# BiaPyX/BiaPy

Hardware: AMD Instinct MI355X
Metric: voxels/sec 3D ResUNet 128^3 patch (train: fwd+bwd+AdamW; sub-records: infer, sliding) (higher is better)
Workload: dtype f16 forward/activations + bf16 gradients (MFMA f16 / bf16, fp32 accumulate)

## Files before the change

biapy_amd/_lib.py:

```python
from __future__ import annotations

import ctypes as C
import os
from typing import Optional

import torch

_HERE = os.path.dirname(os.path.abspath(__file__))
LIB_PATH = os.environ.get("BPX_LIB_PATH") or os.path.join(_HERE, "libbiapy_amd.so")

F32, BF16, F16, U8, MIX16 = 0, 1, 2, 3, 4
U16 = 5
I32 = 6
ACT = {"none": 0, "linear": 0, "elu": 1, "relu": 2, "silu": 3, "leaky_relu": 4, "gelu": 5, "tanh": 6, "sigmoid": 7, "softplus": 8}
PK_K3, PK_K3_T, PK_K1, PK_DENSE, PK_DENSE_T, PK_CT, PK_CT_T, PK_CT4, PK_CT4_T = range(9)


class AxisGrid(C.Structure):
    _fields_ = [("n", C.c_int32), ("step", C.c_int32), ("last", C.c_int32), ("patch", C.c_int32), ("limit", C.c_int32)]


class Tensor(C.Structure):
    _fields_ = [("ptr", C.c_void_p), ("ld", C.c_int32), ("C", C.c_int32), ("cs", C.c_int64)]

# ... 104 lines not shown
    "bpx_debug_set_wgrad_k1": ([_i], _i),
    "bpx_debug_set_pw_stream": ([_i], _i),
    "bpx_debug_set_convt_k1": ([_i], _i),
    "bpx_debug_set_c1_persist": ([_i], _i),
    "bpx_convT3d_k2s2_wgrad_workspace": ([_i, _i, _i, _i, _i, _i, _i], _i64),
    "bpx_conv1x1_fwd": ([_i, _i, _i64, Tensor, _vp, _vp, Tensor, Tensor, _vp, Tensor, Tensor, _vp], _i),
    "bpx_conv1x1_fwd_split_wgrad_workspace": ([_i, _i, _i64, _i], _i64),
    "bpx_conv1x1_fwd_split_wgrad_query": ([_i, _i, _i64, Tensor, Tensor, Tensor, _vp, Tensor, Tensor], _i64),
    "bpx_conv1x1_fwd_split_wgrad": ([_i, _i, _i64, Tensor, _vp, Tensor, Tensor, _vp, Tensor, Tensor, _vp, _vp, _i64, _vp], _i),
    "bpx_conv1x1_fwd_split": ([_i, _i, _i64, Tensor, _vp, _vp, Tensor, Tensor, _vp, Tensor, Tensor, Tensor, _vp], _i),
    "bpx_convT3d_k2s2_fwd": ([_i, _i, _i, _i, _i, _i, Tensor, _vp, _vp, Tensor, _vp, _vp], _i),
    "bpx_convT3d_stats_tiles": ([_i, _i, _i, _i], _i),
    "bpx_convT3d_k2s2_dgrad": ([_i, _i, _i, _i, _i, _i, Tensor, _vp, Tensor, _vp], _i),
    "bpx_convT3d_k2s2_wgrad": ([_i, _i, _i, _i, _i, _i, Tensor, Tensor, _vp, _vp, _vp, _i64, _vp], _i),
    "bpx_convT3d_k2s2_bwd": ([_i, _i, _i, _i, _i, _i, Tensor, Tensor, _vp, Tensor, _vp, _vp, _vp, _i64, _vp], _i),
    "bpx_debug_set_convt_bwd": ([_i], _i),
    "bpx_debug_convt_bwd_launches": ([], _i),
    "bpx_norm_finalize": ([_vp, _i, _i, _i, _i64, _vp, _vp, _f, _i, _vp, _i, _i, _vp], _i),
    "bpx_norm_channel_sums": ([_vp, _i, _i, _i, _vp, _i, _i, _vp], _i),
    "bpx_groupnorm_finalize": ([_vp, _i, _i, _i64, _vp, _vp, _f, _i, _vp, _vp], _i),
    "bpx_groupnorm_bwd_finalize": ([_vp, _i, _i, _i64, _vp, _vp, _vp, _vp, _i, _vp, _vp], _i),
    "bpx_tensor_stats": ([_i, _i, _i64, Tensor, _vp, _vp], _i),
    "bpx_tensor_stats_tiles": ([_i64], _i),
    "bpx_norm_bwd_finalize": ([_vp, _i, _i, _i, _i64, _vp, _vp, _vp, _vp, _i, _vp, _vp], _i),
    "bpx_norm_bwd_finalize_deferred": ([_vp, _i, _i, _i, _i64, _vp, _vp, _vp, _vp, _i, _vp, _vp], _i),
    "bpx_batchnorm_finalize": ([_vp, _i, _i, _i, _i64, _vp, _vp, _f, _f, _vp, _vp, _vp, _vp, _i, _i, _vp], _i),
    "bpx_batchnorm_bwd_finalize": ([_vp, _i, _i, _i, _i64, _vp, _vp, _vp, _vp, _i, _vp, _vp], _i),
    "bpx_batchnorm_eval_records": ([_i, _vp, _i, _vp], _i),
    "bpx_gather3d_tables": ([_vp, _i, _i, _i, _i, _i, _vp, _i, _i, _i, _i, _vp, _vp], _i),
    "bpx_scatter3d_tables": ([_vp, _i, _vp, _i, _i, _i, _i, _vp, _i, _i, _i, _i, _vp], _i),
    "bpx_scatter3d_regions": ([_vp, _i, _i, _i, _i, _i, _vp, _vp, _i, _i, _i, _vp], _i),
    "bpx_wgrad_defer_begin": ([], _i),
    "bpx_wgrad_defer_flush": ([_vp], _i),
    "bpx_norm_bwd_apply": ([_i, _i, _i64, Tensor, Tensor, _vp, Tensor, Tensor, _vp], _i),
    "bpx_channel_affine": ([_i, _i, _i64, Tensor, Tensor, _vp, _vp, Tensor, _vp], _i),
    "bpx_dot_stats": ([_i, _i, _i64, Tensor, Tensor, _vp, _vp], _i),
    "bpx_gate_mlp_fwd": ([_vp, _i, _i, _i, _i64, _vp, _vp, _vp, _vp, _i, _i, _vp, _vp, _vp], _i),
    "bpx_gate_mlp_bwd": ([_vp, _i, _i, _i, _i64, _vp, _vp, _vp, _vp, _i, _i, _vp, _vp, _vp, _vp, _vp, _vp], _i),
    "bpx_norm_act_tiles": ([_i, _i64, _i], _i),
    "bpx_norm_act_dropout_tiles": ([_i, _i64, _i], _i),
    "bpx_norm_act_dropout_fwd": ([_i, _i, _i64, Tensor, _vp, _i, C.c_float, C.c_uint64, _vp, _i, _vp, _i, Tensor, _vp], _i),
    "bpx_norm_act_dropout_bwd": ([_i, _i, _i64, Tensor, Tensor, _vp, _i, C.c_float, C.c_uint64, _vp, _i, _vp, _i, Tensor, _vp, _vp], _i),
    "bpx_norm_act_fwd": ([_i, _i, _i64, Tensor, _vp, _i, Tensor, _vp], _i),
    "bpx_norm_act_bwd": ([_i, _i, _i64, Tensor, Tensor, _vp, _i, Tensor, Tensor, _vp, _vp], _i),
    "bpx_maxpool3d_fwd": ([_i, _i, _i, _i, _i, _i, Tensor, Tensor, _vp, _vp], _i),
    "bpx_maxpool3d_stats_tiles": ([_i, _i, _i, _i, _i, _i], _i),
    "bpx_maxpool3d_bwd_r1_workspace": ([_i, _i, _i, _i, _i, _i, _i], _i64),
    "bpx_maxpool3d_bwd_r1": ([_i, _i, _i, _i, _i, _i, Tensor, Tensor, Tensor, Tensor, _vp, _vp, _vp, _i64, _vp], _i),
    "bpx_maxpool3d_bwd": ([_i, _i, _i, _i, _i, _i, Tensor, Tensor, Tensor, Tensor, _vp], _i),
    "bpx_head_fwd": ([_i, _i64, _i, Tensor, _vp, _vp, _i, _i, _vp, _i64, _i64, _vp], _i),
    "bpx_head_bwd": ([_i, _i64, _i, Tensor, _vp, _i, _vp, _i64, _i64, Tensor, _vp, _vp, _vp, _i64, _vp], _i),
    "bpx_head_bwd_workspace": ([_i, _i], _i64),
    "bpx_conv3d_c1_wgrad_workspace": ([_i], _i64),
    "bpx_conv1x1_c1_wgrad_workspace": ([_i], _i64),
    "bpx_conv3d_c1_fwd": ([_i, _i, _i, _i, _i, _vp, _vp, _vp, Tensor, _vp, _vp], _i),
    "bpx_conv3d_c1_stats_tiles": ([_i, _i, _i], _i),
    "bpx_conv3d_c1_wgrad": ([_i, _i, _i, _i, _i, _vp, Tensor, _vp, _vp, _vp, _i64, _vp], _i),
    "bpx_conv3d_c1_wgrad_nb_supported": ([_i, _i], _i),
    "bpx_conv3d_c1_wgrad_nb": ([_i, _i, _i, _i, _i, _vp, Tensor, Tensor, _vp, _vp, _vp, _vp, _i64, _vp], _i),
    "bpx_conv1x1_c1_wgrad": ([_i, _i64, _vp, Tensor, _vp, _vp, _i64, _vp], _i),
    "bpx_cast": ([_i, _vp, _i, _vp, _i64, _vp], _i),
    "bpx_image_pack16": ([_i, _i, _i64, _i, _vp, _i64, _i64, _i64, _vp, _vp], _i),
    "bpx_upsample_c1_fwd": ([_i, _i, _i, _i, _i, _i, _i, _i, _vp, _vp, _vp, _vp, _vp], _i),
    "bpx_upsample_c1_blocks": ([_i64], _i),
    "bpx_upsample_c1_bwd": ([_i, _i, _i, _i, _i, _i, _i, _i, _vp, _vp, _vp, _vp], _i),
}

EXPORTS = tuple(_SIGS.keys())


class BpxError(RuntimeError):
    pass


def _load() -> C.CDLL:
    if not os.path.exists(LIB_PATH):
        raise ImportError(
            f"{LIB_PATH} is missing: the HIP extension is the product and there is no fallback. "
            "Build it with `python -c 'import __graft_entry__ as g; g.build()'` or `make -C biapy_amd/csrc`."
        )
    lib = C.CDLL(LIB_PATH)
    for name, (args, res) in _SIGS.items():
        fn = getattr(lib, name)
        fn.argtypes = args
        fn.restype = res
    for env, hook in (("BPX_WGRAD_CAP", "bpx_debug_set_wgrad_cap"), ("BPX_WGRAD_K1", "bpx_debug_set_wgrad_k1"),
                      ("BPX_PW_STREAM", "bpx_debug_set_pw_stream"), ("BPX_C1_PERSIST", "bpx_debug_set_c1_persist"),
                      ("BPX_BWD_RS", "bpx_debug_set_bwd_rs"), ("BPX_FUSED_BITS", "bpx_debug_set_bwd_fused"),
                      ("BPX_CT_BWD", "bpx_debug_set_convt_bwd"), ("BPX_LABEL_TILED", "bpx_debug_set_label_tiled"),
                      ("BPX_OVERLAP_PER_VOXEL", "bpx_debug_set_overlap_per_voxel"),
                      ("BPX_REGIONPROPS_LOCAL", "bpx_debug_set_regionprops_local")):
        if os.environ.get(env) is not None:
            getattr(lib, hook)(int(os.environ[env]))
    return lib


class PackJob(C.Structure):
    _fields_ = [("w_d", C.c_void_p), ("packed_d", C.c_void_p), ("mode", C.c_int32), ("Cin", C.c_int32), ("Cout", C.c_int32),
                ("reserved", C.c_int32)]


class BnEvalJob(C.Structure):
    _fields_ = [("gamma_d", C.c_void_p), ("beta_d", C.c_void_p), ("running_mean_d", C.c_void_p), ("running_var_d", C.c_void_p), ("out_d", C.c_void_p),
                ("C", C.c_int32), ("eps", C.c_float)]


class AugCfg(C.Structure):
    _fields_ = [("seed", C.c_uint64), ("thr", C.c_uint64), ("enable", C.c_uint32), ("box_lo", C.c_int32), ("box_hi", C.c_int32),
                ("c_lo", C.c_float), ("c_hi", C.c_float), ("b_lo", C.c_float), ("b_hi", C.c_float), ("s_lo", C.c_float), ("s_hi", C.c_float),
                ("f_lo", C.c_float), ("f_hi", C.c_float)]


class WarpCfg(C.Structure):
    _fields_ = [("seed", C.c_uint64), ("thr", C.c_uint64), ("enable", C.c_uint32), ("reserved", C.c_uint32), ("rot_lo", C.c_float),
                ("rot_hi", C.c_float), ("zoom_lo", C.c_float), ("zoom_hi", C.c_float), ("shear_lo", C.c_float), ("shear_hi", C.c_float),
                ("shift_lo", C.c_float), ("shift_hi", C.c_float)]


class PatchVol(C.Structure):
    _fields_ = [("img", C.c_void_p), ("tgt", C.c_void_p), ("cls", C.c_void_p), ("Z", C.c_int32), ("Y", C.c_int32), ("X", C.c_int32),
                ("reserved", C.c_int32), ("row0", C.c_int64)]

# ... 135 lines not shown
```

biapy_amd/csrc/bpx_common.h:

```cpp
#pragma once
#include <hip/hip_runtime.h>
#include <stdint.h>
#include <stdio.h>
#include <string.h>

#include "../../include/biapy_amd.h"

void bpx_set_error(const char* fmt, ...);
#define BPX_FAIL(...)            \
  do {                           \
    bpx_set_error(__VA_ARGS__);  \
    return 1;                    \
  } while (0)
#define BPX_CHECK(cond, ...) \
  do {                       \
    if (!(cond)) BPX_FAIL(__VA_ARGS__); \
  } while (0)
#define BPX_LAUNCH_CHECK(name)                                                         \
  do {                                                                                 \
    hipError_t e__ = hipGetLastError();                                                \
    if (e__ != hipSuccess) BPX_FAIL("%s: launch failed: %s", name, hipGetErrorString(e__)); \
  } while (0)

typedef __attribute__((ext_vector_type(8))) short bf16x8_t;
// ... 168 lines not shown
  return v;
}

template <int ACTK> __device__ __forceinline__ void act_pair(float& a, float& b, int act) {
  if (ACTK == 1) {
    f32x2_t u{a, b};
    f32x2_t w = u * f32x2_t{1.44269504088896341f, 1.44269504088896341f};
    f32x2_t e = f32x2_t{__builtin_amdgcn_exp2f(w[0]), __builtin_amdgcn_exp2f(w[1])} + f32x2_t{-1.f, -1.f};
    a = __builtin_amdgcn_fmed3f(u[0], e[0], 0.f);
    b = __builtin_amdgcn_fmed3f(u[1], e[1], 0.f);
  } else {
    a = bpx_act_rt<false, false>(a, act);
    b = bpx_act_rt<false, false>(b, act);
  }
}

template <typename T> __device__ __forceinline__ f32x4_t mfma_step(const u32x4_t& a, const u32x4_t& b, f32x4_t c);
template <> __device__ __forceinline__ f32x4_t mfma_step<uint16_t>(const u32x4_t& a, const u32x4_t& b, f32x4_t c) {
  return __builtin_amdgcn_mfma_f32_16x16x32_bf16(__builtin_bit_cast(bf16x8_t, a), __builtin_bit_cast(bf16x8_t, b), c, 0, 0, 0);
}
template <> __device__ __forceinline__ f32x4_t mfma_step<f16_t>(const u32x4_t& a, const u32x4_t& b, f32x4_t c) {
  return __builtin_amdgcn_mfma_f32_16x16x32_f16(__builtin_bit_cast(f16x8_t, a), __builtin_bit_cast(f16x8_t, b), c, 0, 0, 0);
}
template <> __device__ __forceinline__ f32x4_t mfma_step<float>(const u32x4_t& a, const u32x4_t& b, f32x4_t c) {
#pragma unroll
  for (int j = 0; j < 4; ++j)
    c = __builtin_amdgcn_mfma_f32_16x16x4f32(__uint_as_float(a[j]), __uint_as_float(b[j]), c, 0, 0, 0);
  return c;
}

__host__ __device__ __forceinline__ int64_t cdiv64(int64_t a, int64_t b) { return (a + b - 1) / b; }
__host__ __device__ __forceinline__ int cdiv(int a, int b) { return (a + b - 1) / b; }

static inline size_t dtype_size(int dt) {
  switch (dt) {
    case BPX_F32: return 4;
    case BPX_BF16: case BPX_F16: return 2;
    case BPX_U8: return 1;
  }
  return 0;
}

namespace bpxred {
bool defer_active();
int reduce_rows(const char* fn, const float* rows, int groups, int64_t stride, int n, float* dst, hipStream_t s);
int reduce_partials(const char* fn, const float* part, float* dw, int groups, int taps, int Cin, int Cout, int64_t si, int64_t sj, int64_t st,
                    const float* dbpart, float* db, int ndb, bool may_defer, hipStream_t s);
int reduce_partials2(const char* fn, const float* part, float* dw, int groups, int taps, int Cin, int Cout, int64_t si, int64_t sj, int64_t st,
                     const float* dbpart, float* db, float* db2, int ndb, bool may_defer, hipStream_t s);
}
```

biapy_amd/csrc/bwd_fused.hip:

```cpp
#include "conv3d_shared.h"
#include "wgrad_shared.h"

using namespace bpxconv;

#ifndef BPX_BWD_OCC1
#define BPX_BWD_OCC1 3
#endif
#ifndef BPX_BWD_LDSW
#define BPX_BWD_LDSW 1
#endif
#ifndef BPX_BWD_RS_WPRIO
#define BPX_BWD_RS_WPRIO 1
#endif

namespace {

#ifdef BPX_TICKET_PROBE
__device__ unsigned g_probe_ticket = 0u, g_probe_last = 0u;
#endif
struct BwdParams {
  int N, D, H, W;
  const void* dy; int dy_ld;
  const void* wT;
  const void* t; int t_ld; int t_cs; int Ct;
// ... 859 lines not shown
      q_live = have;
      BPX_STAMP();
#pragma unroll
      for (int q = 0; q < NP; ++q) piece(q);
      __builtin_amdgcn_sched_barrier(0);
      BPX_STAMP();
      bpxwg::sd_mfma_phase<WW, CT, HY, HX, VB, VB, TV, NKC>(sA, sG, a_base, g_lane, accw[0], want_b);
      BPX_STAMP();
      if (lane == 0) __hip_atomic_fetch_add(wsync, 1u, __ATOMIC_RELAXED, __HIP_MEMORY_SCOPE_WORKGROUP);
    }
    float* pp = p.part + (size_t)blockIdx.x * 27 * Ct * 16;
#pragma unroll
    for (int a = 0; a < 7; ++a) {
      const int tap = 7 * WW + a;
      if (tap >= 27) continue;
#pragma unroll
      for (int c = 0; c < CT; ++c)
#pragma unroll
        for (int r = 0; r < 4; ++r) pp[((size_t)tap * Ct + c * 16 + 4 * g + r) * 16 + j] = accw[0][a][c][r];
    }
    if (want_b && WW == 3 && g == 0) p.dbpart[(size_t)blockIdx.x * 16 + j] = accw[0][6][0][0];
    __builtin_amdgcn_s_waitcnt(0x0F70);
    };
    switch (ww) {
      case 0: w_role(std::integral_constant<int, 0>{}); break;
      case 1: w_role(std::integral_constant<int, 1>{}); break;
      case 2: w_role(std::integral_constant<int, 2>{}); break;
      default: w_role(std::integral_constant<int, 3>{}); break;
    }
  }
#undef BPX_STAMP
}

int cu_count_() {
  static int n = 0;
  if (n == 0) {
    int dev = 0, v = 0;
    if (hipGetDevice(&dev) == hipSuccess && hipDeviceGetAttribute(&v, hipDeviceAttributeMultiprocessorCount, dev) == hipSuccess && v > 0) n = v;
    else n = 256;
  }
  return n;
}

int g_bwd_fused = 1;

#ifndef BPX_BWD_RS_DEFAULT
#define BPX_BWD_RS_DEFAULT 3
#endif
int g_bwd_rs = BPX_BWD_RS_DEFAULT;

struct BwdPlan { int cg, ct, gy, grid, tilesZ, tilesY, tilesX; bool per_wg_rows; bool rs; };
bool bwd_instance(int Ct, int Cdy, BwdPlan& q) {
  q.gy = 1;
  if (Cdy == 16 && Ct == 16) { q.cg = 1; q.ct = 1; }
  else if (Cdy == 16 && Ct == 48) { q.cg = 1; q.ct = 3; }
  else if (Cdy == 32 && (Ct == 16 || Ct == 32)) { q.cg = 2; q.ct = 1; q.gy = Ct / 16; }
  else return false;
  q.rs = q.cg == 1 && ((q.ct == 3 && (g_bwd_rs & 1)) || (q.ct == 1 && (g_bwd_rs & 2)));
  q.per_wg_rows = q.rs || !(q.cg == 1 && q.ct == 3);
  return true;
}
BwdPlan bwd_plan(int N, int D, int H, int W, int Ct, int Cdy) {
  BwdPlan q{};
  bwd_instance(Ct, Cdy, q);
  q.tilesZ = cdiv(D, 4); q.tilesY = cdiv(H, 4); q.tilesX = cdiv(W, 16);
  const int total = N * q.tilesZ * q.tilesY * q.tilesX;
  const int occ = q.rs ? (q.ct == 1 ? 2 : 1) : (q.cg == 1 && q.ct == 1) ? BPX_BWD_OCC1 : 2;
  int gx = std::max(8, (cu_count_() * occ / std::max(1, q.gy)) & ~7);
  gx = std::min(gx, 8 * cdiv(total, 8));
  q.grid = gx;
  return q;
}

int g_bwd_level1 = 1;

// ... 89 lines not shown
```

biapy_amd/csrc/wgrad.hip:

```cpp
#include <algorithm>
#include <type_traits>
#include <vector>

#include "conv3d_shared.h"
#include "wgrad_shared.h"

namespace {
using bpxwg::sd_mfma_phase;

struct WgradParams {
  int N, D, H, W;
  const void* x; int x_ld; int Cin; const bpx_norm_rec* in_norm; int act;
  int x_cs;
  int x_f16;
  const void* dy; int dy_ld; int Cout; int dy_vs; int dy_oz, dy_oy, dy_ox;
  int dy_vz;
  float* part;
  float* dw; int64_t si, sj, st; int64_t off;
  float* db;
  float* dbpart;
  float* db2;
  int tilesY, tilesX, tilesPerSample, totalTiles, groups;
  int tilesZ, stripY, order;
  void* dx; int dx_ld; const void* wT;
// ... 904 lines not shown
}

int g_ct_resident = 1;
struct CtCfg { int ns, groups, totalTiles, tilesY, tilesX, tilesPerSample; };
inline int ct_mc(int N, int D, int H, int W, int sz, int Cin, int Cout) {
  static const int env = getenv("BPX_CT_MC") ? atoi(getenv("BPX_CT_MC")) : 2;
  return (env >= 2 && sz == 2 && (Cin / 16) % 2 == 0 && Cout % 32 == 0 && (int64_t)N * D * H * W >= 262144) ? 2 : 1;
}
inline CtCfg pick_ct(int N, int D, int H, int W, int sz, int Cin, int Cout) {
  CtCfg c;
  c.ns = (Cout % 32 == 0) ? 2 : 1;
  c.tilesY = cdiv(H, 4); c.tilesX = cdiv(W, 16);
  c.tilesPerSample = cdiv(D, 2) * c.tilesY * c.tilesX;
  c.totalTiles = N * c.tilesPerSample;
  const int nchunks = Cin / (16 * ct_mc(N, D, H, W, sz, Cin, Cout)), nb = Cout / (16 * c.ns);
  const int64_t cap = std::max<int64_t>(1, (int64_t)6400000 / ((int64_t)4 * sz * Cin * Cout));
  const int occ = c.ns == 1 ? 4 : 2;
  const int64_t want = g_ct_resident ? (cdiv64((int64_t)256 * occ, nchunks * nb) + 7) & ~7ll : std::max(1, cdiv(2048, nchunks * nb));
  c.groups = (int)std::max<int64_t>(1, std::min<int64_t>(std::min<int64_t>(c.totalTiles, cap), want));
  return c;
}

struct ReduceJob { const float* part; float* dw; int groups, taps, Cin, Cout; int64_t si, sj, st, off; const float* dbpart; float* db; int ndb; float* db2 = nullptr; int64_t db_stride = 0; };

__host__ __device__ inline int reduce_glanes(int groups) {
  int gl = 1;
  while (gl < 32 && gl * 4 < groups) gl <<= 1;
  return gl;
}
inline int reduce_blocks(const ReduceJob& j) {
  return (int)cdiv64((int64_t)j.taps * j.Cin * j.Cout + (j.db ? (j.ndb ? j.ndb : j.Cout) : 0), 4 * (1024 / reduce_glanes(j.groups)));
}

__device__ __forceinline__ void wgrad_reduce_block(const ReduceJob& j, int block) {
  __shared__ f32x4_t red[1024];
  const float* __restrict__ part = j.part;
  const int groups = j.groups;
  const int GL = reduce_glanes(groups), EL = 1024 / GL;
  const int ndb = j.ndb ? j.ndb : j.Cout;
  const int64_t total = (int64_t)j.taps * j.Cin * j.Cout, all = total + (j.db ? ndb : 0);
  const int e = threadIdx.x % EL, gl = threadIdx.x / EL;
  const int64_t idx = ((int64_t)block * EL + e) * 4;
  const float* __restrict__ src = idx < total ? part + idx : j.dbpart + (idx - total);
  const int64_t stride = idx < total ? total : (j.db_stride ? j.db_stride : ndb);
  const int nval = idx >= all ? 0 : (int)(all - idx < 4 ? all - idx : 4);
  const bool vec = nval == 4 && (stride & 3) == 0 && (((uintptr_t)src) & 15) == 0;
  f32x4_t s0 = f32x4_t{0.f, 0.f, 0.f, 0.f}, s1 = s0, s2 = s0, s3 = s0;
  if (vec) {
    int gq = gl;
    for (; gq + 3 * GL < groups; gq += 4 * GL) {
      s0 += *reinterpret_cast<const f32x4_t*>(src + (size_t)gq * stride);
      s1 += *reinterpret_cast<const f32x4_t*>(src + (size_t)(gq + GL) * stride);
      s2 += *reinterpret_cast<const f32x4_t*>(src + (size_t)(gq + 2 * GL) * stride);
      s3 += *reinterpret_cast<const f32x4_t*>(src + (size_t)(gq + 3 * GL) * stride);
    }
    for (; gq < groups; gq += GL) s0 += *reinterpret_cast<const f32x4_t*>(src + (size_t)gq * stride);
  } else if (nval > 0) {
    int gq = gl;
    for (; gq + 3 * GL < groups; gq += 4 * GL) {
      float a[4][4];
#pragma unroll
      for (int u = 0; u < 4; ++u)
#pragma unroll
        for (int k = 0; k < 4; ++k) a[u][k] = k < nval ? src[(size_t)(gq + u * GL) * stride + k] : 0.f;
#pragma unroll
      for (int u = 0; u < 4; ++u)
#pragma unroll
        for (int k = 0; k < 4; ++k) if (k < nval) s0[k] += a[u][k];
    }
    for (; gq < groups; gq += GL)
      for (int k = 0; k < nval; ++k) s0[k] += src[(size_t)gq * stride + k];
  }
  red[gl * EL + e] = (s0 + s1) + (s2 + s3);
  __syncthreads();
  if (gl == 0 && nval > 0) {
    f32x4_t s = red[e];
    for (int q = 1; q < GL; ++q) s += red[q * EL + e];
    for (int k = 0; k < nval; ++k) {
      const int64_t i = idx + k;
      if (i < total) {
        int co = (int)(i % j.Cout), ci = (int)((i / j.Cout) % j.Cin), tap = (int)(i / ((int64_t)j.Cout * j.Cin));
        j.dw[ci * j.si + co * j.sj + tap * j.st + j.off] = s[k];
      } else {
        j.db[i - total] += s[k];
        if (j.db2) j.db2[i - total] += s[k];
      }
    }
  }
}

__global__ void __launch_bounds__(1024) wgrad_reduce_kernel(const ReduceJob j) { wgrad_reduce_block(j, (int)blockIdx.x); }

constexpr int RB_MAX = 32;
struct ReduceBatch { ReduceJob job[RB_MAX]; int first_block[RB_MAX + 1]; int count; };
__global__ void __launch_bounds__(1024) wgrad_reduce_batch_kernel(const ReduceBatch b) {
  int lo = 0, hi = b.count;
  while (hi - lo > 1) {
    const int mid = (lo + hi) >> 1;
    if ((int)blockIdx.x >= b.first_block[mid]) lo = mid; else hi = mid;
  }
  wgrad_reduce_block(b.job[lo], (int)blockIdx.x - b.first_block[lo]);
}

struct DeferState { bool active = false; std::vector<ReduceJob> jobs; };
thread_local DeferState t_defer;

int finish_wgrad(const char* fn, const ReduceJob& j, hipStream_t s) {
  if (t_defer.active) { t_defer.jobs.push_back(j); return 0; }
  wgrad_reduce_kernel<<<reduce_blocks(j), 1024, 0, s>>>(j);
  BPX_LAUNCH_CHECK(fn);
  return 0;
}

struct K1Params {
  const void* x; int x_ld; int x_cs; const void* dy; int dy_ld;
  int Cin, Cout; int64_t voxels; int nblocks; int groups; float* part;
};
__host__ __device__ constexpr int k1_ring(int stage_bytes) { return 4 * stage_bytes <= 131072 ? 4 : 3 * stage_bytes <= 131072 ? 3 : 2; }
__host__ __device__ constexpr int vmcnt_imm(int n) { return (n & 15) | ((n >> 4) << 14) | 0x0F70; }

template <int MC, int NS, int TV, bool XF16>
__global__ void __launch_bounds__(256) wgrad_k1_dma_kernel(const K1Params p) {
  constexpr int VB = 32, SUBS = TV / 32;
  constexpr int A_BYTES = MC * TV * VB, STAGE = (MC + NS) * TV * VB, RING = k1_ring(STAGE);
  constexpr int NI = (MC + NS) * SUBS;
  static_assert(NI % 4 == 0, "every wave issues the same number of DMA instructions per stage");
  constexpr int IPW = NI / 4;
  static_assert((RING - 2) * IPW < 64, "vmcnt range");
  __shared__ __attribute__((aligned(16))) unsigned char smem[RING * STAGE];
  typedef __attribute__((address_space(3))) void* lds_ptr_t;
  typedef __attribute__((address_space(3))) s16x4_t* lds_tr_ptr;
  const int tid = threadIdx.x, lane = tid & 63, wave = tid >> 6;
  const int i = lane & 15, g = lane >> 4;
  const int grp = blockIdx.x;
  const __amdgpu_buffer_rsrc_t rs_x = __builtin_amdgcn_make_buffer_rsrc(const_cast<void*>(p.x), 0, (int)0x80000000u, 0x00020000);
  const __amdgpu_buffer_rsrc_t rs_g = __builtin_amdgcn_make_buffer_rsrc(const_cast<void*>(p.dy), 0, (int)0x80000000u, 0x00020000);
  const uint32_t xvb = (uint32_t)p.x_ld * 2u, gvb = (uint32_t)p.dy_ld * 2u, xcb = (uint32_t)p.x_cs * 2u;
  const uint32_t lane_v = (uint32_t)(lane >> 1), lane_h = (uint32_t)(lane & 1) * 16u;
  const int64_t voxels = p.voxels;
  const int groups = p.groups, nblocks = p.nblocks;
// ... 412 lines not shown
    BPX_LAUNCH_CHECK(fn);
    return finish_wgrad(fn, ReduceJob{p.part, p.dw, groups, 1, p.Cin, p.Cout, p.si, p.sj, p.st, p.off, nullptr, nullptr, 0, nullptr}, s);
  }
  int rc;
  const int64_t vox = (int64_t)p.N * p.D * p.H * p.W;
  const bool sd_ok = dtype == BPX_BF16 && taps == 27 && p.dy_vs == 1 && c.tx == 16 && c.tz == 4 && g_use_tr != 0 &&
                     vox * std::max(p.x_ld, p.dy_ld) < (1ll << 31) && (((uintptr_t)p.in_norm) & 7) == 0 &&
                     !(p.in_norm != nullptr && p.act > BPX_ACT_SILU);
  if (sd_ok && g_wgrad_sd != 0) rc = launch_wgrad_sd(p, c, s);
  else if (dtype == BPX_BF16) rc = (taps == 27) ? launch_wgrad<uint16_t, 27>(p, c, g_use_tr != 0, s) : launch_wgrad<uint16_t, 1>(p, c, g_use_tr != 0, s);
  else rc = (taps == 27) ? launch_wgrad<float, 27>(p, c, false, s) : launch_wgrad<float, 1>(p, c, false, s);
  BPX_CHECK(rc == 0, "%s: no kernel for tile config", fn);
  BPX_LAUNCH_CHECK(fn);
  const float* dbpart = p.db ? p.part + (size_t)c.groups * taps * p.Cin * p.Cout : nullptr;
  return finish_wgrad(fn, ReduceJob{p.part, p.dw, c.groups, taps, p.Cin, p.Cout, p.si, p.sj, p.st, p.off, dbpart, p.db, 0, p.db ? p.db2 : nullptr}, s);
}

}

namespace bpxred {
int reduce_partials(const char* fn, const float* part, float* dw, int groups, int taps, int Cin, int Cout, int64_t si, int64_t sj, int64_t st,
                    const float* dbpart, float* db, int ndb, bool may_defer, hipStream_t s) {
  return reduce_partials2(fn, part, dw, groups, taps, Cin, Cout, si, sj, st, dbpart, db, nullptr, ndb, may_defer, s);
}
bool defer_active() { return t_defer.active; }
int reduce_rows(const char* fn, const float* rows, int groups, int64_t stride, int n, float* dst, hipStream_t s) {
  ReduceJob j{nullptr, nullptr, groups, 0, 0, n, 0, 0, 0, 0, rows, dst, n, nullptr, stride};
  return finish_wgrad(fn, j, s);
}
int reduce_partials2(const char* fn, const float* part, float* dw, int groups, int taps, int Cin, int Cout, int64_t si, int64_t sj, int64_t st,
                     const float* dbpart, float* db, float* db2, int ndb, bool may_defer, hipStream_t s) {
  const ReduceJob j{part, dw, groups, taps, Cin, Cout, si, sj, st, 0, db ? dbpart : nullptr, db, ndb, db ? db2 : nullptr};
  if (may_defer) return finish_wgrad(fn, j, s);
  wgrad_reduce_kernel<<<reduce_blocks(j), 1024, 0, s>>>(j);
  BPX_LAUNCH_CHECK(fn);
  return 0;
}
}

extern "C" int64_t bpx_conv3d_wgrad_workspace(int N, int D, int H, int W, int Cin, int Cout, int k) {
  int taps = k * k * k;
  WCfg c = pick_wcfg(N, D, H, W, Cin, Cout, taps, false);
  int64_t groups = c.groups;
  if (taps == 27) groups = std::max<int64_t>(groups, sdm_plan(N, D, H, W, Cin, Cout).groups);
  if (taps == 1) groups = std::max<int64_t>(groups, 256);
  return groups * ((int64_t)taps * Cin + 1) * Cout * 4;
}
extern "C" int64_t bpx_convT3d_k2s2_wgrad_workspace(int N, int D, int H, int W, int sz, int Cin, int Cout) {
  WCfg c = pick_wcfg(N, D, H, W, Cin, Cout, 1, false);
  CtCfg t = pick_ct(N, D, H, W, sz, Cin, Cout);
  return std::max(std::max((int64_t)c.groups * ((int64_t)Cin + 1) * Cout * 4, (int64_t)t.groups * ((int64_t)4 * sz * Cin + 1) * Cout * 4),
                  (int64_t)256 * ((int64_t)4 * sz * Cin + 1) * Cout * 4);
}

extern "C" int bpx_debug_set_wgrad_tr(int use_tr) {
  g_use_tr = use_tr & 1;
  g_wgrad_sd = (use_tr & 4) ? 1 : (use_tr & 2) ? 0 : -1;
  g_sd_mc = ((use_tr >> 3) & 7) == 4 ? 0 : ((use_tr >> 3) & 3) ? ((use_tr >> 3) & 3) : -1;
  g_ct_resident = ((use_tr >> 6) & 1) ? 0 : 1;
  if ((use_tr >> 7) & 1) { g_k1_wgs = 1024 * (use_tr >> 8) / 100; g_sd_fill = 100; }
  else g_sd_fill = (use_tr >> 8) ? (use_tr >> 8) : 100;
  return 0;
}

extern "C" int bpx_debug_set_tile_order(int bits) { g_sd_order = bits & 1; return 0; }

// ... 120 lines not shown
    p.dw = dw_d; p.si = (int64_t)dy.C * nsub; p.sj = nsub; p.st = 0; p.off = sub;
    p.db = db_d;
    if (run_wgrad(fn, dtype, p, 1, ws_d, ws_bytes, (hipStream_t)stream)) return 1;
  }
  return 0;
}

}

extern "C" int bpx_convT3d_k2s2_wgrad(int dtype, int N, int D, int H, int W, int sz, bpx_tensor x, bpx_tensor dy, float* dw_d, float* db_d,
                                      void* ws_d, int64_t ws_bytes, bpx_stream_t stream) {
  return ct_wgrad_impl("bpx_convT3d_k2s2_wgrad", dtype, N, D, H, W, sz, x, dy, dw_d, db_d, ws_d, ws_bytes, stream, nullptr);
}

extern "C" int bpx_convT3d_k2s2_bwd(int dtype, int N, int D, int H, int W, int sz, bpx_tensor x, bpx_tensor dy, const void* w_packed_T_d, bpx_tensor dx,
                                    float* dw_d, float* db_d, void* ws_d, int64_t ws_bytes, bpx_stream_t stream) {
  CtDgrad dg{dx, w_packed_T_d, false};
  if (ct_wgrad_impl("bpx_convT3d_k2s2_bwd", dtype, N, D, H, W, sz, x, dy, dw_d, db_d, ws_d, ws_bytes, stream, &dg) != 0) return 1;
  if (dg.fused) return 0;
  return bpx_convT3d_k2s2_dgrad(dtype == BPX_MIX16 ? BPX_BF16 : dtype, N, D, H, W, sz, dy, w_packed_T_d, dx, stream);
}
extern "C" int bpx_debug_set_convt_bwd(int on) { g_ct_bwd = on ? 1 : 0; return 0; }
extern "C" int bpx_debug_convt_bwd_launches(void) { return g_ct_bwd_launches; }

extern "C" int bpx_debug_set_wgrad_k1(int on) { g_k1_dma = (on == 1 || on == 3 || on == 7) ? 1 : 0; g_ct_dma = (on == 1 || on == 5 || on == 7) ? 1 : 0; g_ct_dma_all = on == 7; return 0; }
extern "C" int bpx_debug_set_wgrad_cap(int percent) { g_cap_pct = percent > 0 ? percent : 100; return 0; }

extern "C" int bpx_wgrad_defer_begin(void) {
  t_defer.active = true;
  t_defer.jobs.clear();
  return 0;
}

extern "C" int bpx_wgrad_defer_flush(bpx_stream_t stream) {
  const char* fn = "bpx_wgrad_defer_flush";
  std::vector<ReduceJob> jobs;
  jobs.swap(t_defer.jobs);
  t_defer.active = false;
  hipStream_t s = (hipStream_t)stream;
  for (size_t base = 0; base < jobs.size(); base += RB_MAX) {
    ReduceBatch b{};
    b.count = (int)std::min<size_t>(RB_MAX, jobs.size() - base);
    int blocks = 0;
    for (int k = 0; k < b.count; ++k) {
      b.job[k] = jobs[base + k];
      b.first_block[k] = blocks;
      blocks += reduce_blocks(b.job[k]);
    }
    b.first_block[b.count] = blocks;
    if (blocks == 0) continue;
    wgrad_reduce_batch_kernel<<<blocks, 1024, 0, s>>>(b);
    BPX_LAUNCH_CHECK(fn);
  }
  return 0;
}
```

include/biapy_amd.h:

```cpp
#ifndef BIAPY_AMD_H
#define BIAPY_AMD_H

#include <stdint.h>

#ifdef __cplusplus
extern "C" {
#endif

typedef void* bpx_stream_t;

enum bpx_dtype { BPX_F32 = 0, BPX_BF16 = 1, BPX_F16 = 2, BPX_U8 = 3,
                 BPX_MIX16 = 4,
                 BPX_U16 = 5,
                 BPX_I32 = 6 };
enum bpx_act { BPX_ACT_NONE = 0, BPX_ACT_ELU = 1, BPX_ACT_RELU = 2, BPX_ACT_SILU = 3, BPX_ACT_LEAKY_RELU = 4, BPX_ACT_GELU = 5, BPX_ACT_TANH = 6,
               BPX_ACT_SIGMOID = 7, BPX_ACT_SOFTPLUS = 8, BPX_ACT_LAST = 8 };
enum bpx_pad_mode { BPX_PAD_REFLECT = 0, BPX_PAD_ZEROS = 1 };

int bpx_version(void);
const char* bpx_last_error(void);
int bpx_selftest_layouts(float* out_d , bpx_stream_t stream);
int bpx_debug_set_wgrad_tr(int use_tr);
int bpx_debug_set_conv_stamps(void* stamps_d);
int bpx_debug_set_conv_ws(int on);
// ... 76 lines not shown
                   const void* w_packed_d, const float* bias_d, bpx_tensor sc, const void* w_sc_packed_d,
                   const float* bias_sc_d, bpx_tensor y, float* stats_part_d, bpx_stream_t stream);
int bpx_conv3d_stats_tiles(int dtype, int N, int D, int H, int W, int Cout);
int bpx_conv3d_fwd_pool(int dtype, int N, int D, int H, int W, bpx_tensor x, const bpx_norm_rec* in_norm_d, int act,
                        const void* w_packed_d, const float* bias_d, bpx_tensor sc, const void* w_sc_packed_d,
                        const float* bias_sc_d, bpx_tensor y, float* stats_part_d, int pool_sz, bpx_tensor pooled,
                        float* pool_stats_part_d, bpx_stream_t stream);
int bpx_conv3d_fwd_pool_supported(int dtype, int N, int D, int H, int W, int x_ld, int y_ld, int Cout);
int bpx_conv3d_fwd_shuffle(int dtype, int N, int D, int H, int W, bpx_tensor x, const bpx_norm_rec* in_norm_d, int act, const void* w_packed_d,
                           const float* bias_d, int s, bpx_tensor y, bpx_stream_t stream);

int bpx_conv3d_dgrad(int dtype, int N, int D, int H, int W, bpx_tensor dy, const void* w_packed_T_d,
                     bpx_tensor t, const bpx_norm_rec* t_norm_d, int act, bpx_tensor g,
                     float* red_part_d, bpx_stream_t stream);

int64_t bpx_conv3d_wgrad_workspace(int N, int D, int H, int W, int Cin, int Cout, int k);
int bpx_conv3d_wgrad(int dtype, int N, int D, int H, int W, bpx_tensor x, const bpx_norm_rec* in_norm_d, int act,
                     bpx_tensor dy, int k, float* dw_d, float* db_d, void* ws_d, int64_t ws_bytes, bpx_stream_t stream);
int bpx_conv3d_wgrad_db2(int dtype, int N, int D, int H, int W, bpx_tensor x, const bpx_norm_rec* in_norm_d, int act,
                         bpx_tensor dy, int k, float* dw_d, float* db_d, float* db2_d, void* ws_d, int64_t ws_bytes, bpx_stream_t stream);

int bpx_conv3d_bwd_fused_supported(int dtype, int N, int D, int H, int W, int Ct, int Cdy);
int bpx_conv3d_bwd_fused_stats_tiles(int N, int D, int H, int W, int Ct, int Cdy);
int64_t bpx_conv3d_bwd_fused_workspace(int N, int D, int H, int W, int Ct, int Cdy);
int bpx_conv3d_bwd_fused(int dtype, int N, int D, int H, int W, bpx_tensor dy, const void* w_packed_T_d, bpx_tensor t,
                         const bpx_norm_rec* t_norm_d, int act, bpx_tensor g, float* red_part_d, float* dw_d, float* db_d, float* db2_d,
                         void* ws_d, int64_t ws_bytes, bpx_stream_t stream);
int bpx_debug_set_bwd_fused(int bits);
int bpx_debug_set_bwd_rs(int mask);
int bpx_debug_set_conv_kg(int on);

int bpx_wgrad_defer_begin(void);
int bpx_wgrad_defer_flush(bpx_stream_t stream);

typedef struct bpx_nbwd_coef { float a, b, c0, pad; } bpx_nbwd_coef;

int bpx_conv1x1_fwd(int dtype, int N, int64_t voxels, bpx_tensor x, const void* w_packed_d, const float* bias_d,
                    bpx_tensor g, bpx_tensor t, const bpx_nbwd_coef* coef_d, bpx_tensor addend, bpx_tensor y,
                    bpx_stream_t stream);
int bpx_conv1x1_fwd_split(int dtype, int N, int64_t voxels, bpx_tensor x, const void* w_packed_d, const float* bias_d,
                          bpx_tensor g, bpx_tensor t, const bpx_nbwd_coef* coef_d, bpx_tensor addend, bpx_tensor y_lo,
                          bpx_tensor y_hi, bpx_stream_t stream);
int64_t bpx_conv1x1_fwd_split_wgrad_workspace(int dtype, int N, int64_t voxels, int K);
int64_t bpx_conv1x1_fwd_split_wgrad_query(int dtype, int N, int64_t voxels, bpx_tensor x, bpx_tensor g, bpx_tensor t, const void* coef_d,
                                          bpx_tensor y_lo, bpx_tensor y_hi);
int bpx_conv1x1_fwd_split_wgrad(int dtype, int N, int64_t voxels, bpx_tensor x, const void* w_packed_d, bpx_tensor g, bpx_tensor t,
                                const bpx_nbwd_coef* coef_d, bpx_tensor y_lo, bpx_tensor y_hi, float* dw_d, void* ws_d, int64_t ws_bytes,
                                bpx_stream_t stream);

int bpx_convT3d_k2s2_fwd(int dtype, int N, int D, int H, int W, int sz, bpx_tensor x, const void* w_packed_d,
                         const float* bias_d, bpx_tensor y, float* stats_part_d, bpx_stream_t stream);
int bpx_convT3d_stats_tiles(int D, int H, int W, int sz);
int bpx_convT3d_k2s2_dgrad(int dtype, int N, int D, int H, int W, int sz, bpx_tensor dy, const void* w_packed_T_d,
                           bpx_tensor dx, bpx_stream_t stream);
int64_t bpx_convT3d_k2s2_wgrad_workspace(int N, int D, int H, int W, int sz, int Cin, int Cout);
int bpx_convT3d_k2s2_wgrad(int dtype, int N, int D, int H, int W, int sz, bpx_tensor x, bpx_tensor dy,
                           float* dw_d , float* db_d ,
                           void* ws_d, int64_t ws_bytes, bpx_stream_t stream);
int bpx_convT3d_k2s2_bwd(int dtype, int N, int D, int H, int W, int sz, bpx_tensor x, bpx_tensor dy, const void* w_packed_T_d,
                         bpx_tensor dx, float* dw_d, float* db_d, void* ws_d, int64_t ws_bytes, bpx_stream_t stream);
int bpx_debug_set_convt_bwd(int on);
int bpx_debug_convt_bwd_launches(void);

int bpx_norm_finalize(float* stats_part_d, int N, int tiles, int C, int64_t count_per_channel,
                      const float* gamma_d, const float* beta_d, float eps, int groups,
                      bpx_norm_rec* out_d, int out_ld, int out_off, bpx_stream_t stream);
// ... 267 lines not shown
```

Before: 1.045 billion.

## Add opt-in persistent cost-balanced wgrad reduce kernel with prefetched slab loads

Restructures the weight-gradient partial-sum reduction into reusable unit/request/sum/store pieces, software-pipelining the slab loads (prefetching four ahead) and replacing per-element div/mod index math with incremental counters. Adds a persistent reduce kernel, enabled only by a debug bit, that spreads deferred reduce jobs across resident workgroups by an estimated cost and double-buffers shared memory so the next unit's loads overlap the current store. The default path still uses the batch kernel, but the shared block code and the changed launch bounds (1024, 8) also affect it. Debug hooks report flushed jobs and computed shares.

```diff
diff --git a/biapy_amd/_lib.py b/biapy_amd/_lib.py
--- a/biapy_amd/_lib.py
+++ b/biapy_amd/_lib.py
@@ -160,6 +160,9 @@
     "bpx_scatter3d_regions": ([_vp, _i, _i, _i, _i, _i, _vp, _vp, _i, _i, _i, _vp], _i),
     "bpx_wgrad_defer_begin": ([], _i),
     "bpx_wgrad_defer_flush": ([_vp], _i),
+    "bpx_debug_set_wgrad_reduce": ([_i], _i),
+    "bpx_debug_wgrad_flush_jobs": ([_vp, _i], _i),
+    "bpx_debug_wgrad_reduce_shares": ([_vp, _vp, _i, _i, _vp], _i),
     "bpx_norm_bwd_apply": ([_i, _i, _i64, Tensor, Tensor, _vp, Tensor, Tensor, _vp], _i),
     "bpx_channel_affine": ([_i, _i, _i64, Tensor, Tensor, _vp, _vp, Tensor, _vp], _i),
     "bpx_dot_stats": ([_i, _i, _i64, Tensor, Tensor, _vp, _vp], _i),
@@ -215,7 +218,8 @@
     for env, hook in (("BPX_WGRAD_CAP", "bpx_debug_set_wgrad_cap"), ("BPX_WGRAD_K1", "bpx_debug_set_wgrad_k1"),
                       ("BPX_PW_STREAM", "bpx_debug_set_pw_stream"), ("BPX_C1_PERSIST", "bpx_debug_set_c1_persist"),
                       ("BPX_BWD_RS", "bpx_debug_set_bwd_rs"), ("BPX_FUSED_BITS", "bpx_debug_set_bwd_fused"),
-                      ("BPX_CT_BWD", "bpx_debug_set_convt_bwd"), ("BPX_LABEL_TILED", "bpx_debug_set_label_tiled"),
+                      ("BPX_CT_BWD", "bpx_debug_set_convt_bwd"), ("BPX_WGRAD_REDUCE", "bpx_debug_set_wgrad_reduce"),
+                      ("BPX_LABEL_TILED", "bpx_debug_set_label_tiled"),
                       ("BPX_OVERLAP_PER_VOXEL", "bpx_debug_set_overlap_per_voxel"),
                       ("BPX_REGIONPROPS_LOCAL", "bpx_debug_set_regionprops_local")):
         if os.environ.get(env) is not None:
diff --git a/biapy_amd/csrc/bpx_common.h b/biapy_amd/csrc/bpx_common.h
--- a/biapy_amd/csrc/bpx_common.h
+++ b/biapy_amd/csrc/bpx_common.h
@@ -224,6 +224,8 @@
 __host__ __device__ __forceinline__ int64_t cdiv64(int64_t a, int64_t b) { return (a + b - 1) / b; }
 __host__ __device__ __forceinline__ int cdiv(int a, int b) { return (a + b - 1) / b; }
 
+int cu_count_();
+
 static inline size_t dtype_size(int dt) {
   switch (dt) {
     case BPX_F32: return 4;
diff --git a/biapy_amd/csrc/bwd_fused.hip b/biapy_amd/csrc/bwd_fused.hip
--- a/biapy_amd/csrc/bwd_fused.hip
+++ b/biapy_amd/csrc/bwd_fused.hip
@@ -915,6 +915,7 @@
 #undef BPX_STAMP
 }
 
+}
 int cu_count_() {
   static int n = 0;
   if (n == 0) {
@@ -924,6 +925,7 @@
   }
   return n;
 }
+namespace {
 
 int g_bwd_fused = 1;
 
diff --git a/biapy_amd/csrc/wgrad.hip b/biapy_amd/csrc/wgrad.hip
--- a/biapy_amd/csrc/wgrad.hip
+++ b/biapy_amd/csrc/wgrad.hip
@@ -960,55 +960,105 @@
   return (int)cdiv64((int64_t)j.taps * j.Cin * j.Cout + (j.db ? (j.ndb ? j.ndb : j.Cout) : 0), 4 * (1024 / reduce_glanes(j.groups)));
 }
 
-__device__ __forceinline__ void wgrad_reduce_block(const ReduceJob& j, int block) {
-  __shared__ f32x4_t red[1024];
-  const float* __restrict__ part = j.part;
-  const int groups = j.groups;
-  const int GL = reduce_glanes(groups), EL = 1024 / GL;
+struct ReduceUnit {
+  const float* src;
+  int64_t step;
+  int nval;
+  int slabs;
+  int vec;
+  int pad;
+};
+
+__device__ __forceinline__ ReduceUnit reduce_unit(const ReduceJob& j, int block) {
+  const int lg = __builtin_ctz(reduce_glanes(j.groups)), GL = 1 << lg, EL = 1024 >> lg;
   const int ndb = j.ndb ? j.ndb : j.Cout;
   const int64_t total = (int64_t)j.taps * j.Cin * j.Cout, all = total + (j.db ? ndb : 0);
-  const int e = threadIdx.x % EL, gl = threadIdx.x / EL;
+  const int e = threadIdx.x & (EL - 1), gl = threadIdx.x >> (10 - lg);
+  ReduceUnit u;
   const int64_t idx = ((int64_t)block * EL + e) * 4;
-  const float* __restrict__ src = idx < total ? part + idx : j.dbpart + (idx - total);
+  const float* src = idx < total ? j.part + idx : j.dbpart + (idx - total);
   const int64_t stride = idx < total ? total : (j.db_stride ? j.db_stride : ndb);
+  u.nval = idx >= all ? 0 : (int)(all - idx < 4 ? all - idx : 4);
+  u.vec = u.nval == 4 && (stride & 3) == 0 && (((uintptr_t)src) & 15) == 0;
+  u.pad = 0;
+  u.src = src + (int64_t)gl * stride;
+  u.step = (int64_t)GL * stride;
+  u.slabs = u.nval > 0 ? (j.groups - gl + GL - 1) >> lg : 0;
+  return u;
+}
+
+__device__ __forceinline__ void reduce_request(f32x4_t (&a)[4], const float* __restrict__ p, int64_t step, int n) {
+#pragma unroll
+  for (int q = 0; q < 4; ++q, p += step)
+    a[q] = q < n ? *reinterpret_cast<const f32x4_t*>(p) : f32x4_t{0.f, 0.f, 0.f, 0.f};
+}
+__device__ __forceinline__ void reduce_request(f32x4_t (&a)[4], const ReduceUnit& u) { reduce_request(a, u.src, u.step, u.vec ? u.slabs : 0); }
+
+__device__ __forceinline__ f32x4_t reduce_lane_sum(const ReduceUnit& u, f32x4_t (&a)[4]) {
+  f32x4_t s[4];
+#pragma unroll
+  for (int q = 0; q < 4; ++q) s[q] = f32x4_t{0.f, 0.f, 0.f, 0.f};
+  if (u.vec) {
+    const float* __restrict__ p = u.src + 4 * u.step;
+    int n = u.slabs;
+    for (; n >= 8; n -= 4) {
+#pragma unroll
+      for (int q = 0; q < 4; ++q, p += u.step) {
+        s[q] += a[q];
+        a[q] = *reinterpret_cast<const f32x4_t*>(p);
+        __builtin_amdgcn_sched_barrier(0);
+      }
+    }
+    if (n >= 4) {
+#pragma unroll
+      for (int q = 0; q < 4; ++q) s[q] += a[q];
+      n -= 4;
+      reduce_request(a, p, u.step, n);
+    }
+#pragma unroll
+    for (int q = 0; q < 3; ++q)
+      if (q < n) s[0] += a[q];
+  } else if (u.nval > 0) {
+    const float* __restrict__ p = u.src;
+    int n = u.slabs;
+    for (; n >= 4; n -= 4, p += 4 * u.step) {
+      float r[4][4];
+#pragma unroll
+      for (int q = 0; q < 4; ++q)
+#pragma unroll
+        for (int k = 0; k < 4; ++k) r[q][k] = k < u.nval ? p[q * u.step + k] : 0.f;
+#pragma unroll
+      for (int q = 0; q < 4; ++q)
+#pragma unroll
+        for (int k = 0; k < 4; ++k) if (k < u.nval) s[0][k] += r[q][k];
+    }
+    for (; n > 0; --n, p += u.step)
+      for (int k = 0; k < u.nval; ++k) s[0][k] += p[k];
+  }
+  return (s[0] + s[1]) + (s[2] + s[3]);
+}
+
+__device__ __forceinline__ void reduce_store(const ReduceJob& j, int block, const f32x4_t* red) {
+  const int lg = __builtin_ctz(reduce_glanes(j.groups)), GL = 1 << lg, EL = 1024 >> lg;
+  const int e = threadIdx.x & (EL - 1), gl = threadIdx.x >> (10 - lg);
+  const int64_t total = (int64_t)j.taps * j.Cin * j.Cout, all = total + (j.db ? (j.ndb ? j.ndb : j.Cout) : 0);
+  const int64_t idx = ((int64_t)block * EL + e) * 4;
   const int nval = idx >= all ? 0 : (int)(all - idx < 4 ? all - idx : 4);
-  const bool vec = nval == 4 && (stride & 3) == 0 && (((uintptr_t)src) & 15) == 0;
-  f32x4_t s0 = f32x4_t{0.f, 0.f, 0.f, 0.f}, s1 = s0, s2 = s0, s3 = s0;
-  if (vec) {
-    int gq = gl;
-    for (; gq + 3 * GL < groups; gq += 4 * GL) {
-      s0 += *reinterpret_cast<const f32x4_t*>(src + (size_t)gq * stride);
-      s1 += *reinterpret_cast<const f32x4_t*>(src + (size_t)(gq + GL) * stride);
-      s2 += *reinterpret_cast<const f32x4_t*>(src + (size_t)(gq + 2 * GL) * stride);
-      s3 += *reinterpret_cast<const f32x4_t*>(src + (size_t)(gq + 3 * GL) * stride);
-    }
-    for (; gq < groups; gq += GL) s0 += *reinterpret_cast<const f32x4_t*>(src + (size_t)gq * stride);
-  } else if (nval > 0) {
-    int gq = gl;
-    for (; gq + 3 * GL < groups; gq += 4 * GL) {
-      float a[4][4];
-#pragma unroll
-      for (int u = 0; u < 4; ++u)
-#pragma unroll
-        for (int k = 0; k < 4; ++k) a[u][k] = k < nval ? src[(size_t)(gq + u * GL) * stride + k] : 0.f;
-#pragma unroll
-      for (int u = 0; u < 4; ++u)
-#pragma unroll
-        for (int k = 0; k < 4; ++k) if (k < nval) s0[k] += a[u][k];
-    }
-    for (; gq < groups; gq += GL)
-      for (int k = 0; k < nval; ++k) s0[k] += src[(size_t)gq * stride + k];
-  }
-  red[gl * EL + e] = (s0 + s1) + (s2 + s3);
-  __syncthreads();
   if (gl == 0 && nval > 0) {
     f32x4_t s = red[e];
     for (int q = 1; q < GL; ++q) s += red[q * EL + e];
+    int co = 0, ci = 0, tap = 0;
+    if (idx < total) {
+      const uint32_t r = (uint32_t)idx / (uint32_t)j.Cout;
+      co = (int)((uint32_t)idx - r * (uint32_t)j.Cout);
+      tap = (int)(r / (uint32_t)j.Cin);
+      ci = (int)(r - (uint32_t)tap * (uint32_t)j.Cin);
+    }
     for (int k = 0; k < nval; ++k) {
       const int64_t i = idx + k;
       if (i < total) {
-        int co = (int)(i % j.Cout), ci = (int)((i / j.Cout) % j.Cin), tap = (int)(i / ((int64_t)j.Cout * j.Cin));
         j.dw[ci * j.si + co * j.sj + tap * j.st + j.off] = s[k];
+        if (++co == j.Cout) { co = 0; if (++ci == j.Cin) { ci = 0; ++tap; } }
       } else {
         j.db[i - total] += s[k];
         if (j.db2) j.db2[i - total] += s[k];
@@ -1017,11 +1067,21 @@
   }
 }
 
-__global__ void __launch_bounds__(1024) wgrad_reduce_kernel(const ReduceJob j) { wgrad_reduce_block(j, (int)blockIdx.x); }
+__device__ __forceinline__ void wgrad_reduce_block(const ReduceJob& j, int block) {
+  __shared__ f32x4_t red[1024];
+  const ReduceUnit u = reduce_unit(j, block);
+  f32x4_t a[4];
+  reduce_request(a, u);
+  red[threadIdx.x] = reduce_lane_sum(u, a);
+  __syncthreads();
+  reduce_store(j, block, red);
+}
+
+__global__ void __launch_bounds__(1024, 8) wgrad_reduce_kernel(const ReduceJob j) { wgrad_reduce_block(j, (int)blockIdx.x); }
 
 constexpr int RB_MAX = 32;
-struct ReduceBatch { ReduceJob job[RB_MAX]; int first_block[RB_MAX + 1]; int count; };
-__global__ void __launch_bounds__(1024) wgrad_reduce_batch_kernel(const ReduceBatch b) {
+struct ReduceBatch { ReduceJob job[RB_MAX]; int first_block[RB_MAX + 1]; uint32_t first_cost[RB_MAX + 1]; int count; };
+__global__ void __launch_bounds__(1024, 8) wgrad_reduce_batch_kernel(const ReduceBatch b) {
   int lo = 0, hi = b.count;
   while (hi - lo > 1) {
     const int mid = (lo + hi) >> 1;
@@ -1030,10 +1090,57 @@
   wgrad_reduce_block(b.job[lo], (int)blockIdx.x - b.first_block[lo]);
 }
 
-struct DeferState { bool active = false; std::vector<ReduceJob> jobs; };
+__host__ __device__ inline uint32_t reduce_unit_cost(int groups) {
+  const uint32_t gl = (uint32_t)reduce_glanes(groups);
+  return 2 * (((uint32_t)groups + gl - 1) / gl) + 3;
+}
+__host__ __device__ inline uint32_t reduce_share(uint32_t T, uint32_t n, uint32_t w) { return w * (T / n) + (w < T % n ? w : T % n); }
+__host__ __device__ inline int reduce_unit_at(const ReduceBatch& b, uint32_t c) {
+  for (int k = 0; k < b.count; ++k) {
+    if (c >= b.first_cost[k + 1]) continue;
+    const uint32_t uc = reduce_unit_cost(b.job[k].groups);
+    const uint32_t i = c <= b.first_cost[k] ? 0u : (c - b.first_cost[k] + uc - 1) / uc;
+    if (i < (uint32_t)(b.first_block[k + 1] - b.first_block[k])) return b.first_block[k] + (int)i;
+  }
+  return b.first_block[b.count];
+}
+
+__global__ void __launch_bounds__(1024, 8) wgrad_reduce_persist_kernel(const ReduceBatch b) {
+  __shared__ f32x4_t red[2][1024];
+  const uint32_t T = b.first_cost[b.count];
+  int unit = reduce_unit_at(b, reduce_share(T, gridDim.x, blockIdx.x));
+  const int end = reduce_unit_at(b, reduce_share(T, gridDim.x, blockIdx.x + 1));
+  if (unit >= end) return;
+  int k = 0;
+  while (unit >= b.first_block[k + 1]) ++k;
+  int block = unit - b.first_block[k];
+  ReduceUnit cur = reduce_unit(b.job[k], block);
+  f32x4_t a[4];
+  reduce_request(a, cur);
+  for (int buf = 0;; buf ^= 1) {
+    const int kc = k, bc = block;
+    const bool more = unit + 1 < end;
+    ReduceUnit nxt = cur;
+    if (more) {
+      ++unit;
+      while (unit >= b.first_block[k + 1]) ++k;
+      block = unit - b.first_block[k];
+      nxt = reduce_unit(b.job[k], block);
+    }
+    red[buf][threadIdx.x] = reduce_lane_sum(cur, a);
+    __syncthreads();
+    if (more) reduce_request(a, nxt);
+    reduce_store(b.job[kc], bc, red[buf]);
+    if (!more) break;
+    cur = nxt;
+  }
+}
+
+struct DeferState { bool active = false; std::vector<ReduceJob> jobs; std::vector<ReduceJob> flushed; };
 thread_local DeferState t_defer;
 
 int finish_wgrad(const char* fn, const ReduceJob& j, hipStream_t s) {
+  BPX_CHECK((int64_t)j.taps * j.Cin * j.Cout < (1ll << 31), "%s: a weight gradient of 2^31 elements or more", fn);
   if (t_defer.active) { t_defer.jobs.push_back(j); return 0; }
   wgrad_reduce_kernel<<<reduce_blocks(j), 1024, 0, s>>>(j);
   BPX_LAUNCH_CHECK(fn);
@@ -1512,6 +1619,7 @@
                      const float* dbpart, float* db, float* db2, int ndb, bool may_defer, hipStream_t s) {
   const ReduceJob j{part, dw, groups, taps, Cin, Cout, si, sj, st, 0, db ? dbpart : nullptr, db, ndb, db ? db2 : nullptr};
   if (may_defer) return finish_wgrad(fn, j, s);
+  BPX_CHECK((int64_t)taps * Cin * Cout < (1ll << 31), "%s: a weight gradient of 2^31 elements or more", fn);
   wgrad_reduce_kernel<<<reduce_blocks(j), 1024, 0, s>>>(j);
   BPX_LAUNCH_CHECK(fn);
   return 0;
@@ -1698,6 +1806,32 @@
   return 0;
 }
 
+int g_reduce_bits = 0;
+extern "C" int bpx_debug_set_wgrad_reduce(int bits) { g_reduce_bits = bits; return 0; }
+
+static int reduce_resident_wgs() {
+  static int n = 0;
+  if (n == 0) {
+    int occ = 0;
+    if (hipOccupancyMaxActiveBlocksPerMultiprocessor(&occ, wgrad_reduce_persist_kernel, 1024, 0) != hipSuccess || occ < 1) occ = 1;
+    n = occ * cu_count_();
+  }
+  return n;
+}
+
+static uint64_t reduce_batch_tables(ReduceBatch& b, const int* units) {
+  int blocks = 0;
+  uint64_t cost = 0;
+  for (int k = 0; k <= b.count; ++k) {
+    b.first_block[k] = blocks;
+    b.first_cost[k] = (uint32_t)cost;
+    if (k == b.count) break;
+    blocks += units[k];
+    cost += (uint64_t)units[k] * reduce_unit_cost(b.job[k].groups);
+  }
+  return cost;
+}
+
 extern "C" int bpx_wgrad_defer_flush(bpx_stream_t stream) {
   const char* fn = "bpx_wgrad_defer_flush";
   std::vector<ReduceJob> jobs;
@@ -1707,16 +1841,47 @@
   for (size_t base = 0; base < jobs.size(); base += RB_MAX) {
     ReduceBatch b{};
     b.count = (int)std::min<size_t>(RB_MAX, jobs.size() - base);
-    int blocks = 0;
+    int units[RB_MAX];
     for (int k = 0; k < b.count; ++k) {
       b.job[k] = jobs[base + k];
-      b.first_block[k] = blocks;
-      blocks += reduce_blocks(b.job[k]);
-    }
-    b.first_block[b.count] = blocks;
+      units[k] = reduce_blocks(b.job[k]);
+    }
+    const uint64_t cost = reduce_batch_tables(b, units);
+    const int blocks = b.first_block[b.count];
     if (blocks == 0) continue;
-    wgrad_reduce_batch_kernel<<<blocks, 1024, 0, s>>>(b);
+    if ((g_reduce_bits & 1) && cost < (1ull << 31)) {
+      const int wgs = (g_reduce_bits >> 8) > 0 ? (g_reduce_bits >> 8) : std::min(blocks, reduce_resident_wgs());
+      wgrad_reduce_persist_kernel<<<wgs, 1024, 0, s>>>(b);
+    } else {
+      wgrad_reduce_batch_kernel<<<blocks, 1024, 0, s>>>(b);
+    }
     BPX_LAUNCH_CHECK(fn);
   }
+  t_defer.flushed.swap(jobs);
   return 0;
 }
+
+extern "C" int bpx_debug_wgrad_flush_jobs(int64_t* out, int max_jobs) {
+  const std::vector<ReduceJob>& jobs = t_defer.flushed;
+  for (int k = 0; out != nullptr && k < max_jobs && k < (int)jobs.size(); ++k) {
+    const ReduceJob& j = jobs[k];
+    const int64_t row = j.db ? (j.ndb ? j.ndb : j.Cout) : 0;
+    out[6 * k + 0] = j.groups; out[6 * k + 1] = j.taps; out[6 * k + 2] = j.Cin; out[6 * k + 3] = j.Cout; out[6 * k + 4] = row;
+    out[6 * k + 5] = (int64_t)j.groups * ((int64_t)j.taps * j.Cin * j.Cout + row) * 4;
+  }
+  return (int)jobs.size();
+}
+
+extern "C" int bpx_debug_wgrad_reduce_shares(const int* groups, const int* units, int jobs, int wgs, int* first_unit) {
+  if (groups == nullptr || units == nullptr || first_unit == nullptr || jobs < 1 || jobs > RB_MAX || wgs < 1) return -1;
+  ReduceBatch b{};
+  b.count = jobs;
+  for (int k = 0; k < jobs; ++k) {
+    if (groups[k] < 1 || units[k] < 0) return -1;
+    b.job[k].groups = groups[k];
+  }
+  const uint64_t cost = reduce_batch_tables(b, units);
+  if (cost >= (1ull << 31)) return -1;
+  for (int w = 0; w <= wgs; ++w) first_unit[w] = reduce_unit_at(b, reduce_share((uint32_t)cost, (uint32_t)wgs, (uint32_t)w));
+  return b.first_block[jobs];
+}
diff --git a/include/biapy_amd.h b/include/biapy_amd.h
--- a/include/biapy_amd.h
+++ b/include/biapy_amd.h
@@ -132,6 +132,9 @@
 
 int bpx_wgrad_defer_begin(void);
 int bpx_wgrad_defer_flush(bpx_stream_t stream);
+int bpx_debug_set_wgrad_reduce(int bits);
+int bpx_debug_wgrad_reduce_shares(const int* groups, const int* units, int jobs, int wgs, int* first_unit);
+int bpx_debug_wgrad_flush_jobs(int64_t* out, int max_jobs);
 
 typedef struct bpx_nbwd_coef { float a, b, c0, pad; } bpx_nbwd_coef;
 
```

After: 1.040 billion. About the same (-0.5%).
